# yosungho/LineTR

Measured on AMD Instinct MI355X. Metric: line_descriptors_per_sec, higher is better.
Workload: dtype f32 in/out; GEMMs as 6 bf16-split MFMA products, fp32 accumulate (fp32-faithful); 1 GPU; cfg3: 64 pairs/GPU of 640x480, 200 lines/image -> 199 sub-lines x 21 tokens, d_model=256, seeded weights; pairs_per_gpu=64, collective=none

## Files before the change

### linetr_amd/csrc/linetr_net.hip

```cpp
#include <algorithm>
#include <array>
#include <numeric>
#include <set>

#include "lt_handle.h"
#include "lt_gemm.h"
#include "lt_gemm_split.h"
#include "lt_gemm_split16.h"
#include "lt_st_image.h"
#include "lt_gemm_small.h"
#include "lt_model.h"
#include "lt_attn.h"
#include "lt_attn_fused.h"
#include "lt_gemm_ws.h"
#include "lt_tokmlp.h"
#include "lt_token.h"
#include "lt_bntrain.h"

using namespace lt;

namespace {

const char* gemm_class_name(int precision, int tile, const GemmArgs& g, int groups) {
  static const auto names = [] {
// ... 427 lines not shown
    hipLaunchKernelGGL(mlp123_kernel<false>, grid, dim3(256), 0, st, c.p0, c.p1, c.p2, c.rows, rpw, n.cx, n.cy, n.scale, E.W1, E.b1,
                       E.W2.W, E.W2.b, E.W3.W, E.W3.b, out);
  LT_LAUNCH_CHECK();
  return LINETR_OK;
}

TokMlpArgs tok_mlp_args(const LinetrHandle* h, const EncCall& c) {
  const PosEncoder& E = h->enc[c.which];
  const EncNorm n = enc_norm(h->cfg);
  TokMlpArgs a;
  a.p0 = c.p0; a.p1 = c.p1; a.p2 = c.p2; a.rows = c.rows; a.cx = n.cx; a.cy = n.cy; a.scale = n.scale;
  a.W1 = E.W1; a.b1 = E.b1; a.W2st = E.W2.st; a.b2 = E.W2.b; a.W3st = E.W3.st; a.b3 = E.W3.b; a.W4st = E.W4.st; a.b4 = E.W4.b;
  a.Y = c.act[3]; a.ldy = h->cfg.enc_channels[3];
  return a;
}

int pos_encoder(LinetrHandle* h, hipStream_t st, const EncCall& c, bool tok_mlp) {
  const int *ch = h->cfg.enc_channels, e0 = ch[0], e1 = ch[1], e2 = ch[2], e3 = ch[3];
  const PosEncoder& E = h->enc[c.which];
  const auto& kind = ENC_KIND[c.which];
  const int64_t rows = c.rows;
  int e;
  if (tok_mlp) {
    ProfScope ps(h, st, kind.tok_mlp, 2.0 * rows * (kind.in * e0 + e0 * e1 + e1 * e2 + e2 * e3), (double)rows * (kind.in_bytes + 4 * e3));
    return tok_mlp_launch(tok_mlp_args(h, c), c.which == ENC_WORD, st);
  }
  if (fused_mlp_enabled(h->cfg)) {
    ProfScope ps(h, st, kind.mlp123, 2.0 * rows * (kind.in * e0 + e0 * e1 + e1 * e2), (double)rows * (kind.in_bytes + 4 * e2));
    if ((e = enc_mlp123(h, st, c, c.act[2]))) return e;
  } else {
    {
      ProfScope ps(h, st, "mlp_first", 2.0 * rows * kind.in * e0, (double)rows * (kind.in_bytes + 4 * e0));
      if ((e = enc_layer1<true>(h, st, c, c.act[0]))) return e;
    }
    if ((e = run_gemm(h, st, E.W2, (int)rows, {c.act[0], e0}, {c.act[1], e1}, ACT_RELU))) return e;
    if ((e = run_gemm(h, st, E.W3, (int)rows, {c.act[1], e1}, {c.act[2], e2}, ACT_RELU))) return e;
  }
  return run_gemm(h, st, E.W4, (int)rows, {c.act[2], e2}, {c.act[3], e3}, ACT_RELU);
}

int pos_encoder_bn(LinetrHandle* h, hipStream_t st, const EncCall& c, const BnTrain& bt, int64_t& off) {
  const PosEncoder& E = h->enc[c.which];
  const GemmW* const W[4] = {nullptr, &E.W2, &E.W3, &E.W4};
  const int* ch = h->cfg.enc_channels;
  int e;
  for (int i = 0; i < 4; ++i) {
    e = i == 0 ? enc_layer1<false>(h, st, c, c.act[0])
               : run_gemm(h, st, *W[i], (int)c.rows, {c.act[i - 1], ch[i - 1]}, {c.act[i], ch[i]}, ACT_NONE);
    if (e) return e;
    const int layer = 4 * c.which + i;
    if ((e = bn_train_layer(st, bt, c.act[i], c.rows, ch[i], ch[i], h->bn_g[layer], h->bn_b[layer], off))) return e;
    off += 2 * ch[i];
  }
  return LINETR_OK;
}

int pos_encoders(LinetrHandle* h, hipStream_t& st, const TokenStage& ts, const float* sublines, const float* resp,
                 const float* angle_sub, int N, FwdWs& w) {
  const LinetrModelConfig& c = h->cfg;
  const int e0 = c.enc_channels[0], e1 = c.enc_channels[1], e2 = c.enc_channels[2], e3 = c.enc_channels[3];
  const EncCall word{ENC_WORD, ts.cpnt ? ts.cpnt : ts.pnt, ts.cpnt ? ts.cscore : ts.score, nullptr, ts.rows, w.act[ENC_WORD]};
  const EncCall line{ENC_LINE, sublines, resp, angle_sub, N, w.act[ENC_LINE]};
  const int64_t rows = ts.rows;
  int e;
  const bool tok_mlp_ok = fused_mlp_enabled(c) && h->precision == LINETR_PREC_BF16X6 && e0 == 32 && e1 == 64 && e2 == 128 && e3 == 256 &&
                          !LT_XENV("LINETR_NO_TOKMLP");
  auto has_images = [](const PosEncoder& E) { return E.W2.st && E.W3.st && E.W4.st; };
  const bool tok_mlp = tok_mlp_ok && has_images(h->enc[ENC_WORD]), line_mlp = tok_mlp_ok && has_images(h->enc[ENC_LINE]);
  if (ts.bn) {
    int64_t off = 0;
    if ((e = pos_encoder_bn(h, st, word, *ts.bn, off))) return e;
    if ((e = pos_encoder_bn(h, st, line, *ts.bn, off))) return e;
  } else if (tok_mlp && line_mlp && rows > 0 && N > 0) {
    ProfScope ps(h, st, "pos_mlp_dual_bf16x6", 2.0 * rows * (3 * e0 + e0 * e1 + e1 * e2 + e2 * e3) + 2.0 * N * (5 * e0 + e0 * e1 + e1 * e2 + e2 * e3),
                 (double)rows * (12 + 4 * e3) + (double)N * (28 + 4 * e3));
    if ((e = tok_mlp_launch_dual(tok_mlp_args(h, word), tok_mlp_args(h, line), st))) return e;
  } else {
    if ((e = pos_encoder(h, st, word, tok_mlp))) return e;
    if ((e = pos_encoder(h, st, line, line_mlp))) return e;
  }
  return run_gemm(h, st, h->lW5, N, {w.act[ENC_LINE][3], e3}, {w.lpos, D}, ACT_NONE);
}

int cls_pooling(LinetrHandle* h, hipStream_t& st, const TokenStage& ts, int n_images, int N, int T, FwdWs& w) {
  const int64_t rows = ts.rows;
  if (ts.cpnt) {
    const double tap_bytes = std::min((double)n_images * ts.Hc * ts.Wc * D * 4, (double)rows * D * 4 * 4);
    ProfScope ps(h, st, "cls_pool_online", 2.0 * rows * (2.0 * HEADS * D * 2), tap_bytes + (double)rows * D * 4 + (double)N * HEADS * POOLW * 4);
    if (N <= 2048)
      hipLaunchKernelGGL(cls_pool_online_kernel<4>, dim3(N), dim3(256), 0, st, ts.recs, ts.sub2line_g, ts.cpnt,
                         w.act[ENC_WORD][3], ts.first_pad, N, T, ts.nhwc, ts.Hc, ts.Wc, ts.align_corners, h->pool, w.pooled, 0);
    else
      hipLaunchKernelGGL(cls_pool_online_kernel<1>, dim3(cdiv(N, 4)), dim3(256), 0, st, ts.recs, ts.sub2line_g, ts.cpnt,
                         w.act[ENC_WORD][3], ts.first_pad, N, T, ts.nhwc, ts.Hc, ts.Wc, ts.align_corners, h->pool, w.pooled, 1);
    LT_LAUNCH_CHECK();
  } else {
    ProfScope ps(h, st, "cls_pool", 2.0 * rows * (2.0 * HEADS * D * 2), (double)rows * D * 8);
    hipLaunchKernelGGL(cls_pool_kernel, dim3(N), dim3(256), HEADS * (T + 1) * sizeof(float), st, ts.desc, w.act[ENC_WORD][3], T,
                       h->pool, w.pooled);
    LT_LAUNCH_CHECK();
  }
  const GemmGroups heads{HEADS, DH, POOLW, DH};
  return run_gemm(h, st, h->Watt, N, {w.pooled, HEADS * POOLW}, {w.att, D}, ACT_NONE, nullptr, &heads);
}

int sentence(LinetrHandle* h, hipStream_t& st, int N, FwdWs& w) {
  const LinetrModelConfig& c = h->cfg;
  int e;
  {
    NormSpec ns; ns.mode = 1; ns.gamma = h->ln1g; ns.beta = h->ln1b; ns.eps = 1e-6f;
    if ((e = run_gemm_norm(h, st, h->Wfc, N, {w.att, D}, nullptr, w.fc, w.o, ns))) return e;
  }
  if ((e = run_gemm(h, st, h->Wf1, N, {w.o, D}, {w.f1, c.d_inner}, ACT_GELU))) return e;
  NormSpec ns; ns.mode = 1; ns.gamma = h->ln2g; ns.beta = h->ln2b; ns.add2 = w.lpos; ns.eps = 1e-6f;
  return run_gemm_norm(h, st, h->Wf2, N, {w.f1, c.d_inner}, w.o, w.f2, w.zA, ns);
}

enum { SIGK_F32 = 0, SIGK_SMALL = 1, SIGK_SPLIT4 = 2, SIGK_SPLIT8 = 3, SIGK_FUSED = 4 };
struct SigAttnPlan {
  int attn;
  bool fold_next, fused;
  int kernel() const { return fused ? SIGK_FUSED : attn; }
};
SigAttnPlan sig_attn_plan(const LinetrHandle* h, int n_images, int N, int max_n) {
  SigAttnPlan p;
  const bool small_attn = h->precision != LINETR_PREC_F32 && (int64_t)n_images * HEADS * cdiv(max_n, 256) < 64;
  p.attn = h->precision == LINETR_PREC_F32 ? SIGK_F32 : small_attn ? SIGK_SMALL : max_n <= 128 ? SIGK_SPLIT4 : SIGK_SPLIT8;
  p.fold_next = small_attn && N <= SIG_FOLD_MAX_ROWS && !LT_XENV("LINETR_NO_SIG_FOLD");
  p.fused = !p.fold_next && !LT_XENV("LINETR_NO_FUSED_QKV_ATTN") && h->precision == LINETR_PREC_BF16X6 && max_n <= 256 &&
            (int64_t)n_images * HEADS >= 128;
  return p;
}

int sig_attention(LinetrHandle* h, hipStream_t st, int kernel, const float* qkv, int ldq, const int* cu_dev, int n_images, int N,
                  int max_n, double fl, float* msg) {
  if (kernel == SIGK_F32) {
    ProfScope ps(h, st, "sig_attn", fl, (double)N * D * 16);
    hipLaunchKernelGGL(sig_attn_kernel, dim3(n_images, HEADS, cdiv(max_n, ATT_QT)), dim3(256), 0, st, qkv, cu_dev, msg);
  } else {
    ProfScope ps(h, st, "sig_attn_bf16x6", fl, (double)N * D * 16);
    if (kernel == SIGK_SMALL)
      hipLaunchKernelGGL(sig_attn_small_kernel, dim3(n_images, HEADS, cdiv(max_n, 32)), dim3(256), 0, st, qkv, cu_dev, msg, ldq);
    else if (kernel == SIGK_SPLIT4)
      hipLaunchKernelGGL(sig_attn_split_kernel<4>, dim3(n_images, HEADS, cdiv(max_n, ATT_QT)), dim3(256), 0, st, qkv, cu_dev, msg);
    else
      hipLaunchKernelGGL(sig_attn_split_kernel<8>, dim3(n_images, HEADS, cdiv(max_n, 256)), dim3(512), 0, st, qkv, cu_dev, msg);
  }
  LT_LAUNCH_CHECK();
  return LINETR_OK;
}

int sig_qkv_attention(LinetrHandle* h, hipStream_t st, const SigLayer& S, const float* z, const int* cu_dev, int n_images, int N,
                      double attn_fl, float* msg) {
  LT_HIP(allow_dynamic_lds<sig_qkv_attn_kernel>(FQA_LDS));
  ProfScope ps(h, st, "sig_qkv_attn_bf16x6", 2.0 * N * 3.0 * D * D + attn_fl, (double)N * D * 8);
  hipLaunchKernelGGL(sig_qkv_attn_kernel, dim3(n_images, HEADS), dim3(512), FQA_LDS, st, z, S.Wqkv.st, S.Wqkv.b,
                     cu_dev, msg);
  LT_LAUNCH_CHECK();
  return LINETR_OK;
}

int sig_network(LinetrHandle* h, hipStream_t& st, const TokenStage& ts, const int32_t* h_cu, const int* cu_dev, int n_images, int N,
                float* d_line_desc, FwdWs& w) {
  const LinetrModelConfig& c = h->cfg;
  int max_n = 0;
  for (int i = 0; i < n_images; ++i) max_n = std::max(max_n, h_cu[i + 1] - h_cu[i]);
  int e;
  const double attn_fl = attn_flops(h_cu, n_images);
  const int64_t sig_bn_off = 4 * (int64_t)(c.enc_channels[0] + c.enc_channels[1] + c.enc_channels[2] + c.enc_channels[3]);
  const SigAttnPlan plan = sig_attn_plan(h, n_images, N, max_n);
  const bool fold_next = plan.fold_next, fused_qkv_attn = plan.fused;
  float *z = w.zA, *zn = w.zB;
  int ldz = D;
  float *zq = w.zqA, *zq_next = w.zqB;
  const float* qkv = w.qkv;
  int ldq = 3 * D;
  for (size_t l = 0; l < h->sig.size(); ++l) {
    const SigLayer& S = h->sig[l];
    if (fused_qkv_attn && S.Wqkv.st) {
      if ((e = sig_qkv_attention(h, st, S, z, cu_dev, n_images, N, attn_fl, w.msgp))) return e;
    } else {
      if (!fold_next || l == 0)
        if ((e = run_gemm(h, st, S.Wqkv, N, {z, ldz}, {w.qkv, 3 * D}, ACT_NONE))) return e;
      if ((e = sig_attention(h, st, plan.attn, qkv, ldq, cu_dev, n_images, N, max_n, attn_fl, w.msgp))) return e;
    }
    if ((e = run_gemm(h, st, S.W1, N, {z, ldz, w.msgp, D, D}, {w.hid, 2 * D}, ts.bn ? ACT_NONE : ACT_RELU))) return e;
    if (ts.bn && (e = bn_train_layer(st, *ts.bn, w.hid, N, 2 * D, 2 * D, h->bn_g[8 + l], h->bn_b[8 + l], sig_bn_off + (int64_t)l * 4 * D))) return e;
    if (l + 1 == h->sig.size()) break;
    if (fold_next) {
      if ((e = run_gemm(h, st, S.Wnext, N, {z, ldz, w.hid, 2 * D, D}, {zq, 4 * D}, ACT_NONE))) return e;
      z = zq; ldz = 4 * D; qkv = zq + D; ldq = 4 * D;
      std::swap(zq, zq_next);
    } else {
      if ((e = run_gemm(h, st, S.W2, N, {w.hid, 2 * D}, {zn, D}, ACT_NONE, z))) return e;
      std::swap(z, zn);
    }
    if ((e = pipe_boundary(ts.pipe, CUT_SIG0 + (int)l, st))) return e;
  }
  NormSpec l2; l2.mode = 2;
  if (h->sig.empty()) return run_gemm_norm(h, st, h->Wfin, N, {z, D}, nullptr, zn, d_line_desc, l2);
  return run_gemm_norm(h, st, h->Wfin2, N, {z, ldz, w.hid, 2 * D, D}, nullptr, zn, d_line_desc, l2);
}
}

#ifdef LINETR_EXPERIMENTS
#include "lt_x_net.h"
#endif

namespace {
int forward_core(LinetrHandle* h, hipStream_t st, const TokenStage& ts, const float* sublines, const float* resp,
                 const float* angle_sub, const int32_t* h_cu, const int* cu_dev, int n_images, int N, int T,
                 float* d_line_desc, FwdWs& w) {
  int e;
#ifdef LINETR_EXPERIMENTS
  XPath xp;
  if ((e = x_begin(h, st, n_images, N, h_cu, w, xp))) return e;
#endif
  if ((e = pos_encoders(h, st, ts, sublines, resp, angle_sub, N, w))) return e;
  if ((e = pipe_boundary(ts.pipe, CUT_MLP, st))) return e;
  if ((e = cls_pooling(h, st, ts, n_images, N, T, w))) return e;
  if ((e = pipe_boundary(ts.pipe, CUT_POOL, st))) return e;
#ifdef LINETR_EXPERIMENTS
  if (xp != X_NONE) return x_rest(h, st, ts, h_cu, cu_dev, n_images, N, d_line_desc, w, xp);
#endif
  if ((e = sentence(h, st, N, w))) return e;
  if ((e = pipe_boundary(ts.pipe, CUT_SENTENCE, st))) return e;
  return sig_network(h, st, ts, h_cu, cu_dev, n_images, N, d_line_desc, w);
}

int check_cu(const int32_t* h_cu, int n_images) {
  if (!h_cu || n_images < 1) return fail(LINETR_E_ARG, "null / empty cu_sub");
  if (h_cu[0] != 0) return fail(LINETR_E_ARG, "cu_sub[0] != 0");
  for (int i = 0; i < n_images; ++i)
    if (h_cu[i + 1] < h_cu[i]) return fail(LINETR_E_ARG, "cu_sub not monotone");
  return 0;
}

int cu_on_device(const int32_t* h_cu, const int32_t* d_cu, int n_images, const FwdWs& w, hipStream_t st, const int*& cu_dev) {
  cu_dev = d_cu;
  if (cu_dev) return LINETR_OK;
  LT_HIP(hipMemcpyAsync(w.cu, h_cu, (n_images + 1) * sizeof(int), hipMemcpyHostToDevice, st));
  cu_dev = w.cu;
  return LINETR_OK;
}

int forward_dense(LinetrHandle* h, const char* who, const LinetrTokens& tok, const int32_t* h_cu, const int32_t* d_cu, int n_images,
                  int T, float* d_line_desc, void* d_ws, int64_t ws_bytes, hipStream_t st, BnTrain* bt) {
  if (int e = check_cu(h_cu, n_images)) return e;
  const int N = h_cu[n_images];
  if (N <= 0) return LINETR_OK;
  if (!tok.sublines || !tok.pnt || !tok.resp || !tok.angle_sub || !tok.desc || !tok.score || !d_line_desc)
    return fail(LINETR_E_ARG, "%s: null tensor", who);
  if (ws_bytes < (bt ? linetr_forward_train_workspace_bytes(h, N, T) : linetr_forward_workspace_bytes(h, N, T)))
    return fail(LINETR_E_WORKSPACE, "%s: workspace too small", who);
  if ((int64_t)N * T > INT32_MAX / 8) return fail(LINETR_E_ARG, "%s: batch too large", who);
  LT_HIP(hipSetDevice(h->device));
  FwdWs w = fwd_layout(h, N, (int64_t)N * T, std::max(N, 1), (char*)d_ws);
  if (bt) {
    bt->partial = (double*)((char*)d_ws + align_up(w.total, 256));
    bt->affine = (float*)((char*)bt->partial + (int64_t)BN_MAX_BLOCKS * 2 * BN_MAX_CHANNELS * 8);
  }
  const int* cu_dev;
  if (int e = cu_on_device(h_cu, d_cu, n_images, w, st, cu_dev)) return e;
  TokenStage ts;
  ts.pnt = tok.pnt; ts.score = tok.score; ts.desc = tok.desc; ts.rows = (int64_t)N * T;
  ts.bn = bt;
  return forward_core(h, st, ts, tok.sublines, tok.resp, tok.angle_sub, h_cu, cu_dev, n_images, N, T, d_line_desc, w);
}
}

extern "C" int linetr_forward(LinetrHandle* h, const LinetrTokens* tok, const int32_t* h_cu, const int32_t* d_cu,
                              int32_t n_images, int32_t T, float* d_line_desc, void* d_ws, int64_t ws_bytes,
                              void* stream) {
  if (!h || !tok) return fail(LINETR_E_ARG, "forward: null argument");
  if (h->cfg.bn_batch_stats) return fail(LINETR_E_ARG, "forward: a training-mode handle (bn_batch_stats = 1) runs linetr_forward_train only");
  return forward_dense(h, "forward", *tok, h_cu, d_cu, n_images, T, d_line_desc, d_ws, ws_bytes, (hipStream_t)stream, nullptr);
}

extern "C" int64_t linetr_bn_stats_floats(const LinetrHandle* h) {
  if (!h) return -1;
  const LinetrModelConfig& c = h->cfg;
  return 4 * (int64_t)(c.enc_channels[0] + c.enc_channels[1] + c.enc_channels[2] + c.enc_channels[3]) + (int64_t)c.n_sig_layers * 4 * D;
}

extern "C" int64_t linetr_forward_train_workspace_bytes(const LinetrHandle* h, int32_t N, int32_t T) {
  if (!h) return -1;
  return linetr_forward_workspace_bytes(h, N, T) + (int64_t)BN_MAX_BLOCKS * 2 * BN_MAX_CHANNELS * 8 + 2 * BN_MAX_CHANNELS * 4 + 512;
}

extern "C" int linetr_forward_train(LinetrHandle* h, const LinetrTokens* tok, const int32_t* h_cu, const int32_t* d_cu, int32_t n_images,
                                    int32_t T, float momentum, float* d_bn_running, float* d_bn_batch, float* d_line_desc, void* d_ws,
                                    int64_t ws_bytes, void* stream) {
  if (!h || !tok) return fail(LINETR_E_ARG, "forward_train: null argument");
  if (!h->cfg.bn_batch_stats) return fail(LINETR_E_ARG, "forward_train: the handle was created for inference (bn_batch_stats = 0)");
  if (!d_bn_running) return fail(LINETR_E_ARG, "forward_train: null running statistics");
  if (!(momentum >= 0.f && momentum <= 1.f)) return fail(LINETR_E_ARG, "forward_train: momentum out of [0, 1]");
  BnTrain bt;
  bt.running = d_bn_running; bt.batch = d_bn_batch; bt.momentum = momentum;
  return forward_dense(h, "forward_train", *tok, h_cu, d_cu, n_images, T, d_line_desc, d_ws, ws_bytes, (hipStream_t)stream, &bt);
}


namespace {
// ... 236 lines not shown
```

### linetr_amd/csrc/lt_attn_fused.h

```cpp
#pragma once
#include "lt_st_image.h"
#include "lt_attn.h"

namespace lt {

constexpr int FQA_W_BYTES = 3 * 4 * ST_RB;
constexpr int FQA_SLOT = FQA_W_BYTES + 256 * 64;
constexpr int FQA_KEYS = 128;
constexpr int FQA_LDS = 4 * FQA_SLOT;

__global__ __launch_bounds__(512) void sig_qkv_attn_kernel(const float* __restrict__ z ,
                                                           const unsigned char* __restrict__ Wst ,
                                                           const float* __restrict__ bqkv ,
                                                           const int* __restrict__ cu_sub, float* __restrict__ out ) {
  extern __shared__ __attribute__((aligned(1024))) unsigned char fq_smem[];
  const int img = blockIdx.x, head = blockIdx.y;
  const int n0 = cu_sub[img], Ni = cu_sub[img + 1] - n0;
  if (Ni <= 0) return;
  const int tid = threadIdx.x, lane = tid & 63;
  const int wave = __builtin_amdgcn_readfirstlane(tid >> 6);
  const int h2 = lane >> 5, lq = lane & 31;
  const int q = wave * 32 + lq;
  const bool wave_active = wave * 32 < Ni;
  constexpr int RBW = 3 * D / 16, NK = D / 16;

  const int n_dma = wave < 2 ? 5 : 4;
  const unsigned lane16 = lane * 16;
  auto issue_one = [&](int d, int k, int slot) {
    const int x = wave + 8 * d;
    unsigned char* dst = fq_smem + slot * FQA_SLOT + x * 1024;
    if (x < 18) {
      const unsigned char* g = Wst + ((int64_t)k * RBW + (x / 6) * 16 + head * 4) * ST_RB + (x % 6) * 1024;
      LT_GLDS(g + lane16, dst, 0);
    } else {
      int row = (x - 18) * 16 + (lane >> 2);
      row = row < Ni ? row : Ni - 1;
      const float* g = z + (int64_t)(n0 + row) * D + k * 16 + (((lane & 3) - ((lane >> 4) & 3)) & 3) * 4;
      LT_GLDS(g, dst, 0);
    }
  };
  auto issue_step = [&](int k, int slot) {
#pragma unroll
    for (int d = 0; d < 5; ++d)
      if (d < n_dma) issue_one(d, k, slot);
  };
  auto wait_dma = [&](int steps) {
    if (steps <= 0) asm volatile("s_waitcnt vmcnt(0)" ::: "memory");
    else if (wave < 2) {
      if (steps == 1) asm volatile("s_waitcnt vmcnt(5)" ::: "memory");
      else asm volatile("s_waitcnt vmcnt(10)" ::: "memory");
    } else {
      if (steps == 1) asm volatile("s_waitcnt vmcnt(4)" ::: "memory");
      else asm volatile("s_waitcnt vmcnt(8)" ::: "memory");
    }
  };
#pragma unroll
  for (int k = 0; k < 4; ++k) issue_step(k, k);
  f32x16 acc[6];
  {
    const float* bp = bqkv + head * DH + 4 * h2;
#pragma unroll
    for (int i = 0; i < 6; ++i)
#pragma unroll
      for (int bq = 0; bq < 4; ++bq) {
        const f32x4 v = *reinterpret_cast<const f32x4*>(bp + (i >> 1) * D + (i & 1) * 32 + 8 * bq);
#pragma unroll
        for (int c = 0; c < 4; ++c) acc[i][4 * bq + c] = v[c];
      }
  }
  wait_dma(2);
  __builtin_amdgcn_s_barrier();
  asm volatile("" ::: "memory");

  const int lfrag = ((lane >> 4) & 1) * ST_RB + (lane >> 5) * 256 + (lane & 15) * 16;
  const int zrot = (lq >> 2) & 3;
  const int zoff0 = FQA_W_BYTES + (wave * 32 + lq) * 64 + ((2 * h2 + zrot) & 3) * 16;
  const int zoff1 = FQA_W_BYTES + (wave * 32 + lq) * 64 + ((2 * h2 + 1 + zrot) & 3) * 16;
  using Terms = split_terms<3>;
  auto read_w = [&](int k, int i, int p, bf16x8 (&wf)[3]) {
    wf[p] = *reinterpret_cast<const bf16x8*>(fq_smem + (k & 3) * FQA_SLOT + lfrag + ((i >> 1) * 4 + (i & 1) * 2) * ST_RB + p * ST_CHUNK);
  };
  auto split_z = [&](const f32x4& x0, const f32x4& x1, bf16x8 (&zf)[3]) {
    unsigned a[3], b[3], c[3], d[3];
    split_pair<3>(x0[0], x0[1], a); split_pair<3>(x0[2], x0[3], b);
    split_pair<3>(x1[0], x1[1], c); split_pair<3>(x1[2], x1[3], d);
#pragma unroll
    for (int p = 0; p < 3; ++p) {
      union { bf16x8 v; unsigned w[4]; } u;
      u.w[0] = a[p]; u.w[1] = b[p]; u.w[2] = c[p]; u.w[3] = d[p];
      zf[p] = u.v;
    }
  };
  bf16x8 zfA[3], zfB[3], wfA[3], wfB[3];
  {
    const f32x4 x0 = *reinterpret_cast<const f32x4*>(fq_smem + zoff0), x1 = *reinterpret_cast<const f32x4*>(fq_smem + zoff1);
    split_z(x0, x1, zfA);
#pragma unroll
    for (int p = 0; p < 3; ++p) read_w(0, 0, p, wfA);
  }
  auto step = [&](int s, bf16x8 (&zc)[3], bf16x8 (&zn)[3]) {
    f32x4 zr0, zr1;
    const bool more = s + 1 < NK;
#pragma unroll
    for (int m = 0; m < 36; ++m) {
      const int i = m / 6, t = m % 6;
      bf16x8 (&wc)[3] = (i & 1) ? wfB : wfA;
      bf16x8 (&wn)[3] = (i & 1) ? wfA : wfB;
      acc[i] = mfma_split<0>(wc[Terms::pa(t)], zc[Terms::pb(t)], acc[i]);
      if (t < 3) {
        if (i < 5) read_w(s, i + 1, t, wn);
        else read_w(s + 1, 0, t, wn);
      }
      if (m == 3) zr0 = *reinterpret_cast<const f32x4*>(fq_smem + ((s + 1) & 3) * FQA_SLOT + zoff0);
      if (m == 4) zr1 = *reinterpret_cast<const f32x4*>(fq_smem + ((s + 1) & 3) * FQA_SLOT + zoff1);
      if (m == 15) split_z(zr0, zr1, zn);
      if (m >= 18 && m < 23 && s >= 1 && s + 3 < NK) { if (m - 18 < n_dma) issue_one(m - 18, s + 3, (s + 3) & 3); }
      __builtin_amdgcn_sched_barrier(0);
    }
    asm volatile("s_waitcnt lgkmcnt(0)" ::: "memory");
    if (more) {
      wait_dma(s + 3 < NK ? 1 : 0);
      __builtin_amdgcn_s_barrier();
      asm volatile("" ::: "memory");
    }
    __builtin_amdgcn_sched_barrier(0);
  };
#pragma unroll 1
  for (int s = 0; s < NK; s += 2) {
    step(s, zfA, zfB);
    step(s + 1, zfB, zfA);
  }
  asm volatile("s_waitcnt vmcnt(0)" ::: "memory");

  auto pieces = [&](const f32x16& a, float scale, float (&v)[16]) {
#pragma unroll
    for (int r = 0; r < 16; ++r) v[r] = a[r] * scale;
#pragma unroll
    for (int c = 0; c < 4; ++c) { halves_swap(v[c], v[4 + c]); halves_swap(v[8 + c], v[12 + c]); }
  };
  auto split_run = [&](const float* x, bf16x8 (&o)[3]) {
    unsigned a[3], b[3], c[3], d[3];
    split_pair<3>(x[0], x[1], a); split_pair<3>(x[2], x[3], b);
    split_pair<3>(x[4], x[5], c); split_pair<3>(x[6], x[7], d);
#pragma unroll
    for (int p = 0; p < 3; ++p) {
      union { bf16x8 v; unsigned w[4]; } u;
      u.w[0] = a[p]; u.w[1] = b[p]; u.w[2] = c[p]; u.w[3] = d[p];
      o[p] = u.v;
    }
  };
  bf16x8 qf[4][3];
#pragma unroll
  for (int i = 0; i < 2; ++i) {
    float v[16];
    pieces(acc[i], LOG2E, v);
    split_run(v, qf[2 * i]);
    split_run(v + 8, qf[2 * i + 1]);
  }
  unsigned char* Ks = fq_smem;
  unsigned char* Vs = fq_smem + FQA_KEYS * ATS_RK;
  auto stage_kv = [&]() {
    const int r = (wave & 3) * 32 + lq;
#pragma unroll
    for (int i = 2; i < 6; ++i) {
      float v[16];
      pieces(acc[i], 1.f, v);
      unsigned char* dst = (i < 4 ? Ks + r * ATS_RK : Vs + r * ATS_RV) + ((i & 1) * 32 + 8 * h2) * 2;
#pragma unroll
      for (int g = 0; g < 2; ++g) {
        bf16x8 pl[3];
        split_run(v + 8 * g, pl);
#pragma unroll
        for (int p = 0; p < 3; ++p) *reinterpret_cast<bf16x8*>(dst + p * 128 + g * 32) = pl[p];
      }
    }
  };
  f32x16 o0, o1;
#pragma unroll
  for (int r = 0; r < 16; ++r) { o0[r] = 0.f; o1[r] = 0.f; }
  float m = -INFINITY, l = 0.f;
  const unsigned v_base = (unsigned)(size_t)(Vs + (((lane & 15) >> 2) + 4 * h2) * ATS_RV + (((lane >> 4) & 1) * 16 + (lane & 3) * 4) * 2);
  auto chunk = [&](int kv0, auto kv_local) {
    constexpr int KL = decltype(kv_local)::value;
    constexpr int KB = KL >= 64 ? 64 : 0;
    const unsigned vb = v_base + KB * ATS_RV;
    u32x2 vrA[3][2], vrB[3][2];
    v_frags_tr<KL - KB, 0, false>(vb, vrA);
    f32x16 st;
#pragma unroll
    for (int r = 0; r < 16; ++r) st[r] = 0.f;
    const unsigned char* kp = Ks + (KL + lq) * ATS_RK + h2 * 16;
    bf16x8 kaA[3], kaB[3];
#pragma unroll
    for (int p = 0; p < 3; ++p) kaA[p] = *reinterpret_cast<const bf16x8*>(kp + p * 128);
#pragma unroll
    for (int m = 0; m < 24; ++m) {
      const int sq = m / 6, t = m % 6;
      bf16x8 (&kc)[3] = (sq & 1) ? kaB : kaA;
      bf16x8 (&kn)[3] = (sq & 1) ? kaA : kaB;
      st = mfma_split<0>(kc[split_terms<3>::pa(t)], qf[sq][split_terms<3>::pb(t)], st);
      if (t < 3 && sq < 3) kn[t] = *reinterpret_cast<const bf16x8*>(kp + t * 128 + (sq + 1) * 32);
      __builtin_amdgcn_sched_barrier(0);
    }
    if (kv0 + 32 > Ni) {
#pragma unroll
      for (int r = 0; r < 16; ++r)
        if (kv0 + (r & 3) + 8 * (r >> 2) + 4 * h2 >= Ni) st[r] = -INFINITY;
    }
    float mx = st[0];
#pragma unroll
    for (int r = 1; r < 16; ++r) mx = fmaxf(mx, st[r]);
    mx = xor32_max(mx);
    const float m_new = fmaxf(m, mx);
// ... 83 lines not shown
```

### linetr_amd/csrc/lt_gemm.h

```cpp
#pragma once
#include "lt_common.h"

namespace lt {

enum { ACT_NONE = 0, ACT_RELU = 1, ACT_GELU = 2, ACT_DIST = 3  };

struct GemmArgs {
  const float* A;   int lda;
  const float* A2;  int lda2;  int K1;
  const float* W;   int ldw;
  const float* bias;
  const float* R;   int ldr;
  float* Y;         int ldy;
  int M, N, K;
  int act;
  int64_t gA, gW, gBias, gY;
  int norm = 0;
  const float* gamma = nullptr;
  const float* beta = nullptr;
  const float* add2 = nullptr;
  int ldadd2 = 0;
  float eps = 0.f;
};

constexpr int GEMM_BK = 32;
constexpr int GEMM_LDS_STRIDE = GEMM_BK + 4;

__device__ __forceinline__ float apply_act(float v, int act) {
  if (act == ACT_RELU) v = fmaxf(v, 0.f);
  else if (act == ACT_GELU) v = 0.5f * v * (1.f + erff(v * 0.70710678118654752440f));
  else if (act == ACT_DIST) v = fmaxf(2.f - 2.f * v, 0.f);
  return v;
}

__device__ __forceinline__ constexpr int cd_row(int r, int h) { return (r & 3) + 8 * (r >> 2) + 4 * h; }

template <int PL>
struct split_terms {
  static_assert(PL == 2 || PL == 3, "two or three planes");
  static constexpr int N = PL * (PL + 1) / 2;
  static constexpr int PA[6] = {PL == 3 ? 2 : 1, PL == 3 ? 1 : 0, 0, 1, 0, 0};
  static constexpr int PB[6] = {0, 1, PL == 3 ? 2 : 0, 0, 1, 0};
  static constexpr int pa(int t) { return PA[t]; }
  static constexpr int pb(int t) { return PB[t]; }
  static constexpr bool follows_rule() {
    int t = 0;
    for (int ord = PL - 1; ord >= 0; --ord)
      for (int a = PL - 1; a >= 0; --a) {
        if (ord - a < 0 || ord - a >= PL) continue;
        if (PA[t] != a || PB[t] != ord - a) return false;
        ++t;
      }
    return t == N;
  }
};
static_assert(split_terms<2>::follows_rule(), "PL 2: (1,0) (0,1) (0,0)");
static_assert(split_terms<3>::follows_rule(), "PL 3: (2,0) (1,1) (0,2) (1,0) (0,1) (0,0)");

__device__ __forceinline__ int xcd_tile(int block, int ntile) {
  const int b = block, q = ntile / 8, r = ntile % 8, xcd = b % 8, k = b / 8;
  return (xcd < r ? xcd * (q + 1) : r * (q + 1) + (xcd - r) * q) + k;
}

template <int BM, int BN, int WM, int WN>
__global__ __launch_bounds__(256) void gemm_kernel(GemmArgs g) {
  constexpr int TM = BM / WM, TN = BN / WN;
  constexpr int MI = TM / 32, NI = TN / 32;
  static_assert(WM * WN == 4 && MI >= 1 && NI >= 1, "bad tiling");
  constexpr int LS = GEMM_LDS_STRIDE;
  constexpr int A_F4 = BM * 8 / 256;
  constexpr int B_F4 = BN * 8 / 256;
  static_assert(A_F4 >= 1 && B_F4 >= 1, "tile too small");

  extern __shared__ __attribute__((aligned(16))) float smem[];
  float* As = smem;
  float* Bs = smem + 2 * BM * LS;

  const int tid = threadIdx.x, lane = tid & 63, wave = tid >> 6;
  const int wm = wave / WN, wn = wave % WN;
  const int m0 = blockIdx.y * BM, n0 = blockIdx.x * BN;
  const int grp = blockIdx.z;
  const float* A = g.A + grp * g.gA;
  const float* A2 = g.A2 ? g.A2 + grp * g.gA : nullptr;
  const float* W = g.W + grp * g.gW;
  const int K1 = g.A2 ? g.K1 : g.K;

  const int lrow = tid >> 3, lc4 = (tid & 7) * 4;

  f32x4 ra[A_F4], rb[B_F4];
  auto gload = [&](int k0) {
    const float* src = A; int ld = g.lda; int kk = k0;
    if (k0 >= K1) { src = A2; ld = g.lda2; kk = k0 - K1; }
#pragma unroll
    for (int i = 0; i < A_F4; ++i) {
      int r = m0 + lrow + i * 32;
      r = r < g.M ? r : g.M - 1;
      ra[i] = *reinterpret_cast<const f32x4*>(src + (int64_t)r * ld + kk + lc4);
    }
#pragma unroll
    for (int i = 0; i < B_F4; ++i) {
      int r = n0 + lrow + i * 32;
      rb[i] = *reinterpret_cast<const f32x4*>(W + (int64_t)r * g.ldw + k0 + lc4);
    }
  };
  auto lstore = [&](int buf) {
#pragma unroll
    for (int i = 0; i < A_F4; ++i)
      *reinterpret_cast<f32x4*>(&As[(buf * BM + lrow + i * 32) * LS + lc4]) = ra[i];
#pragma unroll
    for (int i = 0; i < B_F4; ++i)
      *reinterpret_cast<f32x4*>(&Bs[(buf * BN + lrow + i * 32) * LS + lc4]) = rb[i];
  };

  f32x16 acc[MI][NI];
#pragma unroll
  for (int i = 0; i < MI; ++i)
#pragma unroll
    for (int j = 0; j < NI; ++j)
#pragma unroll
      for (int r = 0; r < 16; ++r) acc[i][j][r] = 0.f;

  const int nk = g.K / GEMM_BK;
  gload(0);
  lstore(0);
  __syncthreads();
  const int frow = lane & 31, fk = (lane >> 5) * 4;
  for (int kt = 0; kt < nk; ++kt) {
    const int buf = kt & 1;
    if (kt + 1 < nk) gload((kt + 1) * GEMM_BK);
    const float* Ab = &As[(buf * BM + wm * TM + frow) * LS + fk];
    const float* Bb = &Bs[(buf * BN + wn * TN + frow) * LS + fk];
#pragma unroll
    for (int kk = 0; kk < 4; ++kk) {
      f32x4 af[MI], bf[NI];
#pragma unroll
      for (int i = 0; i < MI; ++i) af[i] = *reinterpret_cast<const f32x4*>(Ab + i * 32 * LS + kk * 8);
#pragma unroll
      for (int j = 0; j < NI; ++j) bf[j] = *reinterpret_cast<const f32x4*>(Bb + j * 32 * LS + kk * 8);
#pragma unroll
      for (int s = 0; s < 4; ++s)
#pragma unroll
        for (int i = 0; i < MI; ++i)
#pragma unroll
// ... 66 lines not shown
```

### linetr_amd/csrc/lt_model.h

```cpp
#pragma once
#include "lt_common.h"
#include "lt_token.h"
#include "lt_gemm_split.h"

namespace lt {

template <bool RELU = true>
__global__ void word_mlp1_kernel(const float* __restrict__ pnt, const float* __restrict__ score, int64_t rows,
                                 float cx, float cy, float scale, const float* __restrict__ W ,
                                 const float* __restrict__ b, float* __restrict__ out ) {
#pragma clang fp contract(off)
  const int64_t gid = (int64_t)blockIdx.x * blockDim.x + threadIdx.x;
  const int64_t row = gid >> 3;
  if (row >= rows) return;
  const int c0 = (int)(gid & 7) * 4;
  const float x = (pnt[row * 2 + 0] - cx) / scale;
  const float y = (pnt[row * 2 + 1] - cy) / scale;
  const float s = score[row];
  f32x4 o;
#pragma unroll
  for (int c = 0; c < 4; ++c) {
    const float* w = W + (c0 + c) * 3;
    float v = b[c0 + c] + w[0] * x + w[1] * y + w[2] * s;
    o[c] = RELU ? fmaxf(v, 0.f) : v;
  }
  *reinterpret_cast<f32x4*>(out + row * 32 + c0) = o;
}

template <bool RELU = true>
__global__ void line_mlp1_kernel(const float* __restrict__ sublines , const float* __restrict__ resp,
                                 const float* __restrict__ angle, int N, float cx, float cy, float scale,
                                 const float* __restrict__ W , const float* __restrict__ b,
                                 float* __restrict__ out ) {
#pragma clang fp contract(off)
  const int gid = blockIdx.x * blockDim.x + threadIdx.x;
  const int row = gid >> 3;
  if (row >= N) return;
  const int c0 = (gid & 7) * 4;
  const float* sl = sublines + (int64_t)row * 4;
  const float sx = (sl[0] - cx) / scale, sy = (sl[1] - cy) / scale;
  const float ex = (sl[2] - cx) / scale, ey = (sl[3] - cy) / scale;
  const float in[5] = {(sx + ex) / 2.f, (sy + ey) / 2.f, resp[row], angle[row * 2], angle[row * 2 + 1]};
  f32x4 o;
#pragma unroll
  for (int c = 0; c < 4; ++c) {
    const float* w = W + (c0 + c) * 5;
    float v = b[c0 + c];
#pragma unroll
    for (int i = 0; i < 5; ++i) v += w[i] * in[i];
    o[c] = RELU ? fmaxf(v, 0.f) : v;
  }
  *reinterpret_cast<f32x4*>(out + (int64_t)row * 32 + c0) = o;
}

__device__ __forceinline__ void word_feat(const float* __restrict__ pnt, const float* __restrict__ score, int64_t row,
                                          float cx, float cy, float scale, float (&in)[3]) {
#pragma clang fp contract(off)
  in[0] = (pnt[row * 2 + 0] - cx) / scale;
  in[1] = (pnt[row * 2 + 1] - cy) / scale;
  in[2] = score[row];
}
__device__ __forceinline__ void line_feat(const float* __restrict__ sublines, const float* __restrict__ resp,
                                          const float* __restrict__ angle, int64_t row, float cx, float cy, float scale,
                                          float (&in)[5]) {
#pragma clang fp contract(off)
  const float* sl = sublines + row * 4;
  const float sx = (sl[0] - cx) / scale, sy = (sl[1] - cy) / scale;
  const float ex = (sl[2] - cx) / scale, ey = (sl[3] - cy) / scale;
  in[0] = (sx + ex) / 2.f; in[1] = (sy + ey) / 2.f; in[2] = resp[row]; in[3] = angle[row * 2]; in[4] = angle[row * 2 + 1];
}

template <bool WORD>
__global__ __launch_bounds__(256) void mlp123_kernel(const float* __restrict__ p0, const float* __restrict__ p1,
                                                     const float* __restrict__ p2, int64_t rows, int rows_per_wave,
                                                     float cx, float cy, float scale,
                                                     const float* __restrict__ W1 , const float* __restrict__ b1,
                                                     const float* __restrict__ W2 , const float* __restrict__ b2,
                                                     const float* __restrict__ W3 , const float* __restrict__ b3,
                                                     float* __restrict__ out ) {
  constexpr int IN = WORD ? 3 : 5;
  const int lane = threadIdx.x & 63, col = lane & 31, h = lane >> 5;
  const int64_t wave = (int64_t)blockIdx.x * 4 + (threadIdx.x >> 6);
  const int64_t r_begin = wave * rows_per_wave;
// ... 106 lines not shown
          for (int q = 0; q < 2; ++q)
            acc3[q] = __builtin_amdgcn_mfma_f32_32x32x2f32(w3[2 * jp + q][i * 16 + r], acc2[i][r], acc3[q], 0, 0, 0);
#pragma unroll
      for (int q = 0; q < 2; ++q)
#pragma unroll
        for (int r = 0; r < 16; r += 4)
          *reinterpret_cast<f32x4*>(stg + col * 68 + 32 * q + cd_row(r, h)) =
              f32x4{fmaxf(acc3[q][r], 0.f), fmaxf(acc3[q][r + 1], 0.f), fmaxf(acc3[q][r + 2], 0.f), fmaxf(acc3[q][r + 3], 0.f)};
      __builtin_amdgcn_wave_barrier();
#pragma unroll
      for (int i = 0; i < 8; ++i) {
        const int t = 4 * i + (lane >> 4), pc = (lane & 15) * 4;
        if (base + t < r_end)
          *reinterpret_cast<f32x4*>(out + (base + t) * 128 + 64 * jp + pc) = *reinterpret_cast<const f32x4*>(stg + t * 68 + pc);
      }
      __builtin_amdgcn_wave_barrier();
    }
#pragma unroll
    for (int i = 0; i < IN; ++i) feat[i] = feat_next[i];
  }
}


__global__ __launch_bounds__(256) void cls_pool_kernel(const float* __restrict__ desc ,
                                                       const float* __restrict__ a4 , int T,
                                                       ClsPoolConst cc, float* __restrict__ pooled ) {
  extern __shared__ float sm[];
  const int S = T + 1;
  const int n = blockIdx.x;
  const int tid = threadIdx.x, lane = tid & 63, wave = tid >> 6;
  const float* dn = desc + (int64_t)n * T * D;
  const float* an = a4 + (int64_t)n * T * D;
  f32x4 u[4], u2[4];
#pragma unroll
  for (int h = 0; h < 4; ++h) {
    u[h] = *reinterpret_cast<const f32x4*>(cc.U + h * D + lane * 4);
    u2[h] = *reinterpret_cast<const f32x4*>(cc.U2 + h * D + lane * 4);
  }
  for (int j = wave; j < T; j += 4) {
    const f32x4 dv = *reinterpret_cast<const f32x4*>(dn + j * D + lane * 4);
    const f32x4 av = *reinterpret_cast<const f32x4*>(an + j * D + lane * 4);
#pragma unroll
    for (int h = 0; h < 4; ++h) {
      float p = 0.f;
#pragma unroll
      for (int c = 0; c < 4; ++c) p += dv[c] * u[h][c] + av[c] * u2[h][c];
      p = wave_sum(p);
      if (lane == 0) sm[h * S + 1 + j] = p + cc.c_tok[h];
    }
  }
  if (tid < 4) sm[tid * S] = cc.s_cls[tid];
  __syncthreads();
  if (tid < 4) {
    float* s = sm + tid * S;
    float mx = s[0];
    for (int j = 1; j < S; ++j) mx = fmaxf(mx, s[j]);
    float sum = 0.f;
    for (int j = 0; j < S; ++j) { s[j] = expf(s[j] - mx); sum += s[j]; }
    for (int j = 0; j < S; ++j) s[j] = s[j] / sum;
  }
  __syncthreads();
  float db[4] = {0.f, 0.f, 0.f, 0.f}, ab[4] = {0.f, 0.f, 0.f, 0.f};
  for (int j = 0; j < T; ++j) {
    const float dv = dn[j * D + tid], av = an[j * D + tid];
#pragma unroll
    for (int h = 0; h < 4; ++h) {
      const float p = sm[h * S + 1 + j];
      db[h] += p * dv;
      ab[h] += p * av;
    }
  }
  float* out = pooled + (int64_t)n * 4 * POOLW;
#pragma unroll
  for (int h = 0; h < 4; ++h) {
    out[h * POOLW + tid] = db[h];
    out[h * POOLW + 256 + tid] = ab[h];
  }
  if (tid < 4 * 32) {
    const int h = tid >> 5, i = tid & 31;
    out[h * POOLW + 512 + i] = i == 0 ? sm[h * S] : 0.f;
  }
}

template <int SPLIT>
__global__ __launch_bounds__(256, 3) void cls_pool_online_kernel(
    const LinetrLineRec* __restrict__ recs, const int* __restrict__ sub2line_g, const float* __restrict__ cpnt,
    const float* __restrict__ a4, int64_t first_pad, int N, int T, const float* __restrict__ nhwc, int Hc, int Wc,
    int align_corners, ClsPoolConst cc, float* __restrict__ pooled , int reverse) {
  const int lane = threadIdx.x & 63;
  const int wv = threadIdx.x >> 6;
  const int n_fwd = SPLIT == 1 ? blockIdx.x * 4 + wv : blockIdx.x;
  if (n_fwd >= N) return;
  const int n = reverse ? N - 1 - n_fwd : n_fwd;
  const LinetrLineRec r = recs[sub2line_g[n]];
  const int j = n - r.first_sub;
  const int n_valid = min(T, r.n_tok - j * T);
  const int n_pad = T - n_valid;
  const int ntk = n_valid + (n_pad > 0 ? 1 : 0);
  const int64_t tok0 = (int64_t)r.first_tok + (int64_t)j * T;
  const int64_t padrow = first_pad + r.image;
  const float* nhwc_img = nhwc + (int64_t)r.image * Hc * Wc * D;
  f32x4 u[4], u2[4];
#pragma unroll
  for (int h = 0; h < 4; ++h) {
    u[h] = *reinterpret_cast<const f32x4*>(cc.U + h * D + lane * 4);
    u2[h] = *reinterpret_cast<const f32x4*>(cc.U2 + h * D + lane * 4);
  }
  float m[4], l[4], w0[4];
  f32x4 db[4], ab[4];
#pragma unroll
  for (int h = 0; h < 4; ++h) {
    m[h] = cc.s_cls[h] * LOG2E; l[h] = 1.f; w0[h] = 1.f;
    if (SPLIT > 1 && wv != 0) { m[h] = -INFINITY; l[h] = 0.f; w0[h] = 0.f; }
    db[h] = f32x4{0.f, 0.f, 0.f, 0.f};
    ab[h] = f32x4{0.f, 0.f, 0.f, 0.f};
  }
  auto row_of = [&](int jj) -> int64_t { return jj < n_valid ? tok0 + jj : padrow; };
  int t_off[4];
  float t_w[4];
  auto fill_taps = [&](int chunk) {
    const int jj = chunk + lane;
    const int64_t row = row_of(jj < ntk ? jj : ntk - 1);
    tap_coords(cpnt[row * 2], cpnt[row * 2 + 1], Hc, Wc, align_corners, t_off, t_w);
  };
  auto issue = [&](int jj, TapSet& t, f32x4& a) {
    int off[4];
    float wt[4];
#pragma unroll
    for (int k = 0; k < 4; ++k) {
      off[k] = __builtin_amdgcn_readlane(t_off[k], jj & 63);
      wt[k] = __builtin_bit_cast(float, __builtin_amdgcn_readlane(__builtin_bit_cast(int, t_w[k]), jj & 63));
    }
    taps_load(nhwc_img, off, wt, lane, t);
    a = *reinterpret_cast<const f32x4*>(a4 + row_of(jj) * D + lane * 4);
  };
  TapSet cur, nxt;
  f32x4 a_cur, a_nxt;
  const int jj0 = SPLIT == 1 ? 0 : wv;
  fill_taps(0);
  if (jj0 < ntk) issue(jj0, cur, a_cur);
  for (int jj = jj0; jj < ntk; jj += SPLIT) {
    if (jj + SPLIT < ntk) {
      if (((jj + SPLIT) >> 6) != (jj >> 6)) fill_taps((jj + SPLIT) & ~63);
      issue(jj + SPLIT, nxt, a_nxt);
    }
    const f32x4 dv = taps_finish<true>(cur);
    const float mult = jj < n_valid ? 1.f : (float)n_pad;
    float sc[4];
#pragma unroll
    for (int h = 0; h < 4; ++h) {
      float p = 0.f;
#pragma unroll
      for (int c = 0; c < 4; ++c) p += dv[c] * u[h][c] + a_cur[c] * u2[h][c];
      sc[h] = p;
    }
    wave_sum_n<4>(sc);
#pragma unroll
    for (int h = 0; h < 4; ++h) {
      const float sh = (sc[h] + cc.c_tok[h]) * LOG2E;
      if (__any(sh > m[h])) {
        const float alpha = __builtin_amdgcn_exp2f(m[h] - sh);
        m[h] = sh;
        l[h] *= alpha;
        w0[h] *= alpha;
#pragma unroll
        for (int c = 0; c < 4; ++c) { db[h][c] *= alpha; ab[h][c] *= alpha; }
      }
      const float e = __builtin_amdgcn_exp2f(sh - m[h]) * mult;
      l[h] += e;
#pragma unroll
      for (int c = 0; c < 4; ++c) {
        db[h][c] += e * dv[c];
        ab[h][c] += e * a_cur[c];
      }
    }
    cur = nxt;
// ... 92 lines not shown
```

Baseline: 10.21 million line-descriptors/s.

## Map pooling blocks to XCD-local image runs and skip idle-wave attention math

The pooling kernel's SPLIT=1 path now gives each XCD a contiguous range of whole images, split at image boundaries, and walks that range in reverse. The aim is to keep each image's NHWC feature map and token activations resident in that XCD's L2 and to keep the tail ordering of the old reversed launch. In the fused QKV-attention kernel, inactive waves no longer run the MFMA steps; they only join the DMA issue and barriers. Uneven image counts per XCD can leave some XCDs with more blocks and cause load imbalance.

```diff
diff --git a/linetr_amd/csrc/linetr_net.hip b/linetr_amd/csrc/linetr_net.hip
--- a/linetr_amd/csrc/linetr_net.hip
+++ b/linetr_amd/csrc/linetr_net.hip
@@ -533,17 +533,18 @@
   return run_gemm(h, st, h->lW5, N, {w.act[ENC_LINE][3], e3}, {w.lpos, D}, ACT_NONE);
 }
 
-int cls_pooling(LinetrHandle* h, hipStream_t& st, const TokenStage& ts, int n_images, int N, int T, FwdWs& w) {
+int cls_pooling(LinetrHandle* h, hipStream_t& st, const TokenStage& ts, const int32_t* h_cu, int n_images, int N, int T, FwdWs& w) {
   const int64_t rows = ts.rows;
   if (ts.cpnt) {
     const double tap_bytes = std::min((double)n_images * ts.Hc * ts.Wc * D * 4, (double)rows * D * 4 * 4);
     ProfScope ps(h, st, "cls_pool_online", 2.0 * rows * (2.0 * HEADS * D * 2), tap_bytes + (double)rows * D * 4 + (double)N * HEADS * POOLW * 4);
+    const PoolRuns runs = pool_runs(h_cu, n_images);
     if (N <= 2048)
       hipLaunchKernelGGL(cls_pool_online_kernel<4>, dim3(N), dim3(256), 0, st, ts.recs, ts.sub2line_g, ts.cpnt,
-                         w.act[ENC_WORD][3], ts.first_pad, N, T, ts.nhwc, ts.Hc, ts.Wc, ts.align_corners, h->pool, w.pooled, 0);
+                         w.act[ENC_WORD][3], ts.first_pad, N, T, ts.nhwc, ts.Hc, ts.Wc, ts.align_corners, h->pool, w.pooled, runs);
     else
-      hipLaunchKernelGGL(cls_pool_online_kernel<1>, dim3(cdiv(N, 4)), dim3(256), 0, st, ts.recs, ts.sub2line_g, ts.cpnt,
-                         w.act[ENC_WORD][3], ts.first_pad, N, T, ts.nhwc, ts.Hc, ts.Wc, ts.align_corners, h->pool, w.pooled, 1);
+      hipLaunchKernelGGL(cls_pool_online_kernel<1>, dim3(runs.blocks(4)), dim3(256), 0, st, ts.recs, ts.sub2line_g, ts.cpnt,
+                         w.act[ENC_WORD][3], ts.first_pad, N, T, ts.nhwc, ts.Hc, ts.Wc, ts.align_corners, h->pool, w.pooled, runs);
     LT_LAUNCH_CHECK();
   } else {
     ProfScope ps(h, st, "cls_pool", 2.0 * rows * (2.0 * HEADS * D * 2), (double)rows * D * 8);
@@ -669,7 +670,7 @@
 #endif
   if ((e = pos_encoders(h, st, ts, sublines, resp, angle_sub, N, w))) return e;
   if ((e = pipe_boundary(ts.pipe, CUT_MLP, st))) return e;
-  if ((e = cls_pooling(h, st, ts, n_images, N, T, w))) return e;
+  if ((e = cls_pooling(h, st, ts, h_cu, n_images, N, T, w))) return e;
   if ((e = pipe_boundary(ts.pipe, CUT_POOL, st))) return e;
 #ifdef LINETR_EXPERIMENTS
   if (xp != X_NONE) return x_rest(h, st, ts, h_cu, cu_dev, n_images, N, d_line_desc, w, xp);
diff --git a/linetr_amd/csrc/lt_attn_fused.h b/linetr_amd/csrc/lt_attn_fused.h
--- a/linetr_amd/csrc/lt_attn_fused.h
+++ b/linetr_amd/csrc/lt_attn_fused.h
@@ -92,7 +92,7 @@
     }
   };
   bf16x8 zfA[3], zfB[3], wfA[3], wfB[3];
-  {
+  if (wave_active) {
     const f32x4 x0 = *reinterpret_cast<const f32x4*>(fq_smem + zoff0), x1 = *reinterpret_cast<const f32x4*>(fq_smem + zoff1);
     split_z(x0, x1, zfA);
 #pragma unroll
@@ -125,10 +125,23 @@
     }
     __builtin_amdgcn_sched_barrier(0);
   };
+  auto idle_step = [&](int s) {
+    if (s >= 1 && s + 3 < NK) issue_step(s + 3, (s + 3) & 3);
+    if (s + 1 < NK) {
+      wait_dma(s + 3 < NK ? 1 : 0);
+      __builtin_amdgcn_s_barrier();
+      asm volatile("" ::: "memory");
+    }
+  };
+  if (wave_active) {
 #pragma unroll 1
-  for (int s = 0; s < NK; s += 2) {
-    step(s, zfA, zfB);
-    step(s + 1, zfB, zfA);
+    for (int s = 0; s < NK; s += 2) {
+      step(s, zfA, zfB);
+      step(s + 1, zfB, zfA);
+    }
+  } else {
+#pragma unroll 1
+    for (int s = 0; s < NK; ++s) idle_step(s);
   }
   asm volatile("s_waitcnt vmcnt(0)" ::: "memory");
 
diff --git a/linetr_amd/csrc/lt_gemm.h b/linetr_amd/csrc/lt_gemm.h
--- a/linetr_amd/csrc/lt_gemm.h
+++ b/linetr_amd/csrc/lt_gemm.h
@@ -57,8 +57,11 @@
 static_assert(split_terms<2>::follows_rule(), "PL 2: (1,0) (0,1) (0,0)");
 static_assert(split_terms<3>::follows_rule(), "PL 3: (2,0) (1,1) (0,2) (1,0) (0,1) (0,0)");
 
+constexpr int XCDS = 8;
+__host__ __device__ __forceinline__ int xcd_of(int block) { return block % XCDS; }
+__host__ __device__ __forceinline__ int xcd_slot(int block) { return block / XCDS; }
 __device__ __forceinline__ int xcd_tile(int block, int ntile) {
-  const int b = block, q = ntile / 8, r = ntile % 8, xcd = b % 8, k = b / 8;
+  const int q = ntile / XCDS, r = ntile % XCDS, xcd = xcd_of(block), k = xcd_slot(block);
   return (xcd < r ? xcd * (q + 1) : r * (q + 1) + (xcd - r) * q) + k;
 }
 
diff --git a/linetr_amd/csrc/lt_model.h b/linetr_amd/csrc/lt_model.h
--- a/linetr_amd/csrc/lt_model.h
+++ b/linetr_amd/csrc/lt_model.h
@@ -1,4 +1,6 @@
 #pragma once
+#include <algorithm>
+
 #include "lt_common.h"
 #include "lt_token.h"
 #include "lt_gemm_split.h"
@@ -271,16 +273,35 @@
   }
 }
 
+
+struct PoolRuns {
+  int s[XCDS + 1];
+  int blocks(int per_block) const {
+    int longest = 0;
+    for (int x = 0; x < XCDS; ++x) longest = std::max(longest, s[x + 1] - s[x]);
+    return XCDS * cdiv(longest, per_block);
+  }
+};
+inline PoolRuns pool_runs(const int32_t* h_cu, int n_images) {
+  PoolRuns r;
+  const int64_t N = h_cu[n_images];
+  for (int x = 0; x <= XCDS; ++x) r.s[x] = *std::lower_bound(h_cu, h_cu + n_images, (int32_t)(x * N / XCDS));
+  return r;
+}
+
 template <int SPLIT>
 __global__ __launch_bounds__(256, 3) void cls_pool_online_kernel(
     const LinetrLineRec* __restrict__ recs, const int* __restrict__ sub2line_g, const float* __restrict__ cpnt,
     const float* __restrict__ a4, int64_t first_pad, int N, int T, const float* __restrict__ nhwc, int Hc, int Wc,
-    int align_corners, ClsPoolConst cc, float* __restrict__ pooled , int reverse) {
+    int align_corners, ClsPoolConst cc, float* __restrict__ pooled , PoolRuns runs ) {
   const int lane = threadIdx.x & 63;
   const int wv = threadIdx.x >> 6;
-  const int n_fwd = SPLIT == 1 ? blockIdx.x * 4 + wv : blockIdx.x;
-  if (n_fwd >= N) return;
-  const int n = reverse ? N - 1 - n_fwd : n_fwd;
+  int n = blockIdx.x;
+  if constexpr (SPLIT == 1) {
+    const int x = xcd_of(blockIdx.x);
+    n = runs.s[x + 1] - 1 - (xcd_slot(blockIdx.x) * 4 + wv);
+    if (n < runs.s[x]) return;
+  }
   const LinetrLineRec r = recs[sub2line_g[n]];
   const int j = n - r.first_sub;
   const int n_valid = min(T, r.n_tok - j * T);
```

After: 10.28 million line-descriptors/s, median of 6. About the same (+0.7%).
